# pythoncrazy/jimm

Measured on NVIDIA H100. Metric: images/sec, higher is better.
Workload: dtype f16

## Files before the change

jimm_b200/csrc/common.cuh:

```cuda
#pragma once

#include <cuda.h>
#include <cuda_bf16.h>
#include <cuda_fp16.h>
#include <cuda_runtime.h>
#include <stdint.h>

namespace jimm {

void set_last_error(const char* fmt, ...);

#define JIMM_CUDA_CHECK(expr)                                                                   \
  do {                                                                                          \
    cudaError_t _e = (expr);                                                                    \
    if (_e != cudaSuccess) {                                                                    \
      ::jimm::set_last_error("%s:%d: %s -> %s", __FILE__, __LINE__, #expr, cudaGetErrorString(_e)); \
      return -2;                                                                                \
    }                                                                                           \
  } while (0)

void note_launch();
#define JIMM_LAUNCH_CHECK()                  \
  do {                                       \
    JIMM_CUDA_CHECK(cudaGetLastError());     \
// ... 156 lines not shown
}
__device__ __forceinline__ void mbar_arrive_cluster(uint32_t cluster_addr) {
  asm volatile("mbarrier.arrive.release.cluster.shared::cluster.b64 _, [%0];" ::"r"(cluster_addr) : "memory");
}
__device__ __forceinline__ uint64_t make_wgmma_desc_sw128(uint32_t smem_addr) {
  uint64_t d = 0;
  d |= static_cast<uint64_t>((smem_addr & 0x3FFFFu) >> 4);
  d |= static_cast<uint64_t>(1) << 16;
  d |= static_cast<uint64_t>(1024 >> 4) << 32;
  d |= static_cast<uint64_t>(1) << 62;
  return d;
}
template <int SW>
__device__ __forceinline__ uint64_t make_wgmma_desc(uint32_t smem_addr, uint32_t lbo) {
  static_assert(SW == 128 || SW == 64 || SW == 32, "swizzle width");
  constexpr uint64_t layout = SW == 128 ? 1 : SW == 64 ? 2 : 3;
  uint64_t d = 0;
  d |= static_cast<uint64_t>((smem_addr & 0x3FFFFu) >> 4);
  d |= static_cast<uint64_t>((lbo >> 4) & 0x3FFFu) << 16;
  d |= static_cast<uint64_t>(8 * SW >> 4) << 32;
  d |= layout << 62;
  return d;
}
__device__ __forceinline__ void wgmma_fence() { asm volatile("wgmma.fence.sync.aligned;" ::: "memory"); }
__device__ __forceinline__ void wgmma_commit() { asm volatile("wgmma.commit_group.sync.aligned;" ::: "memory"); }
template <int N>
__device__ __forceinline__ void wgmma_wait() { asm volatile("wgmma.wait_group.sync.aligned %0;" ::"n"(N) : "memory"); }
template <int R>
__device__ __forceinline__ void wgmma_fence_operands(float (&d)[R]) {
#pragma unroll
  for (int i = 0; i < R; ++i) asm volatile("" : "+f"(d[i])::"memory");
}

template <int KIND>
__device__ __forceinline__ void wgmma_m64n128_ss(float (&d)[64], uint64_t adesc, uint64_t bdesc, uint32_t accumulate) {
  if constexpr (KIND == 0) {
    asm volatile(
        "{\n\t.reg .pred p;\n\t"
        "setp.ne.b32 p, %66, 0;\n\t"
        "wgmma.mma_async.sync.aligned.m64n128k16.f32.f16.f16 {%0, %1, %2, %3, %4, %5, %6, %7, %8, %9, %10, %11, %12, %13, %14, %15, %16, %17, %18, %19, %20, %21, %22, %23, %24, %25, %26, %27, %28, %29, %30, %31, %32, %33, %34, %35, %36, %37, %38, %39, %40, %41, %42, %43, %44, %45, %46, %47, %48, %49, %50, %51, %52, %53, %54, %55, %56, %57, %58, %59, %60, %61, %62, %63}, %64, %65, p, 1, 1, 0, 0;\n\t}"
        : "+f"(d[0]), "+f"(d[1]), "+f"(d[2]), "+f"(d[3]), "+f"(d[4]), "+f"(d[5]), "+f"(d[6]), "+f"(d[7]),
          "+f"(d[8]), "+f"(d[9]), "+f"(d[10]), "+f"(d[11]), "+f"(d[12]), "+f"(d[13]), "+f"(d[14]), "+f"(d[15]),
          "+f"(d[16]), "+f"(d[17]), "+f"(d[18]), "+f"(d[19]), "+f"(d[20]), "+f"(d[21]), "+f"(d[22]), "+f"(d[23]),
          "+f"(d[24]), "+f"(d[25]), "+f"(d[26]), "+f"(d[27]), "+f"(d[28]), "+f"(d[29]), "+f"(d[30]), "+f"(d[31]),
          "+f"(d[32]), "+f"(d[33]), "+f"(d[34]), "+f"(d[35]), "+f"(d[36]), "+f"(d[37]), "+f"(d[38]), "+f"(d[39]),
          "+f"(d[40]), "+f"(d[41]), "+f"(d[42]), "+f"(d[43]), "+f"(d[44]), "+f"(d[45]), "+f"(d[46]), "+f"(d[47]),
          "+f"(d[48]), "+f"(d[49]), "+f"(d[50]), "+f"(d[51]), "+f"(d[52]), "+f"(d[53]), "+f"(d[54]), "+f"(d[55]),
          "+f"(d[56]), "+f"(d[57]), "+f"(d[58]), "+f"(d[59]), "+f"(d[60]), "+f"(d[61]), "+f"(d[62]), "+f"(d[63])
        : "l"(adesc), "l"(bdesc), "r"(accumulate));
  } else if constexpr (KIND == 1) {
    asm volatile(
        "{\n\t.reg .pred p;\n\t"
        "setp.ne.b32 p, %66, 0;\n\t"
        "wgmma.mma_async.sync.aligned.m64n128k16.f32.bf16.bf16 {%0, %1, %2, %3, %4, %5, %6, %7, %8, %9, %10, %11, %12, %13, %14, %15, %16, %17, %18, %19, %20, %21, %22, %23, %24, %25, %26, %27, %28, %29, %30, %31, %32, %33, %34, %35, %36, %37, %38, %39, %40, %41, %42, %43, %44, %45, %46, %47, %48, %49, %50, %51, %52, %53, %54, %55, %56, %57, %58, %59, %60, %61, %62, %63}, %64, %65, p, 1, 1, 0, 0;\n\t}"
        : "+f"(d[0]), "+f"(d[1]), "+f"(d[2]), "+f"(d[3]), "+f"(d[4]), "+f"(d[5]), "+f"(d[6]), "+f"(d[7]),
          "+f"(d[8]), "+f"(d[9]), "+f"(d[10]), "+f"(d[11]), "+f"(d[12]), "+f"(d[13]), "+f"(d[14]), "+f"(d[15]),
          "+f"(d[16]), "+f"(d[17]), "+f"(d[18]), "+f"(d[19]), "+f"(d[20]), "+f"(d[21]), "+f"(d[22]), "+f"(d[23]),
          "+f"(d[24]), "+f"(d[25]), "+f"(d[26]), "+f"(d[27]), "+f"(d[28]), "+f"(d[29]), "+f"(d[30]), "+f"(d[31]),
          "+f"(d[32]), "+f"(d[33]), "+f"(d[34]), "+f"(d[35]), "+f"(d[36]), "+f"(d[37]), "+f"(d[38]), "+f"(d[39]),
          "+f"(d[40]), "+f"(d[41]), "+f"(d[42]), "+f"(d[43]), "+f"(d[44]), "+f"(d[45]), "+f"(d[46]), "+f"(d[47]),
          "+f"(d[48]), "+f"(d[49]), "+f"(d[50]), "+f"(d[51]), "+f"(d[52]), "+f"(d[53]), "+f"(d[54]), "+f"(d[55]),
          "+f"(d[56]), "+f"(d[57]), "+f"(d[58]), "+f"(d[59]), "+f"(d[60]), "+f"(d[61]), "+f"(d[62]), "+f"(d[63])
        : "l"(adesc), "l"(bdesc), "r"(accumulate));
  } else {
    asm volatile(
        "{\n\t.reg .pred p;\n\t"
        "setp.ne.b32 p, %66, 0;\n\t"
        "wgmma.mma_async.sync.aligned.m64n128k8.f32.tf32.tf32 {%0, %1, %2, %3, %4, %5, %6, %7, %8, %9, %10, %11, %12, %13, %14, %15, %16, %17, %18, %19, %20, %21, %22, %23, %24, %25, %26, %27, %28, %29, %30, %31, %32, %33, %34, %35, %36, %37, %38, %39, %40, %41, %42, %43, %44, %45, %46, %47, %48, %49, %50, %51, %52, %53, %54, %55, %56, %57, %58, %59, %60, %61, %62, %63}, %64, %65, p, 1, 1;\n\t}"
        : "+f"(d[0]), "+f"(d[1]), "+f"(d[2]), "+f"(d[3]), "+f"(d[4]), "+f"(d[5]), "+f"(d[6]), "+f"(d[7]),
          "+f"(d[8]), "+f"(d[9]), "+f"(d[10]), "+f"(d[11]), "+f"(d[12]), "+f"(d[13]), "+f"(d[14]), "+f"(d[15]),
          "+f"(d[16]), "+f"(d[17]), "+f"(d[18]), "+f"(d[19]), "+f"(d[20]), "+f"(d[21]), "+f"(d[22]), "+f"(d[23]),
          "+f"(d[24]), "+f"(d[25]), "+f"(d[26]), "+f"(d[27]), "+f"(d[28]), "+f"(d[29]), "+f"(d[30]), "+f"(d[31]),
          "+f"(d[32]), "+f"(d[33]), "+f"(d[34]), "+f"(d[35]), "+f"(d[36]), "+f"(d[37]), "+f"(d[38]), "+f"(d[39]),
          "+f"(d[40]), "+f"(d[41]), "+f"(d[42]), "+f"(d[43]), "+f"(d[44]), "+f"(d[45]), "+f"(d[46]), "+f"(d[47]),
          "+f"(d[48]), "+f"(d[49]), "+f"(d[50]), "+f"(d[51]), "+f"(d[52]), "+f"(d[53]), "+f"(d[54]), "+f"(d[55]),
          "+f"(d[56]), "+f"(d[57]), "+f"(d[58]), "+f"(d[59]), "+f"(d[60]), "+f"(d[61]), "+f"(d[62]), "+f"(d[63])
        : "l"(adesc), "l"(bdesc), "r"(accumulate));
  }
}

template <bool BF16>
__device__ __forceinline__ void wgmma_m64n64k16_ss(float (&d)[32], uint64_t adesc, uint64_t bdesc, uint32_t accumulate) {
  if constexpr (BF16) {
    asm volatile(
        "{\n\t.reg .pred p;\n\t"
        "setp.ne.b32 p, %34, 0;\n\t"
        "wgmma.mma_async.sync.aligned.m64n64k16.f32.bf16.bf16 {%0, %1, %2, %3, %4, %5, %6, %7, %8, %9, %10, %11, %12, %13, %14, %15, %16, %17, %18, %19, %20, %21, %22, %23, %24, %25, %26, %27, %28, %29, %30, %31}, %32, %33, p, 1, 1, 0, 0;\n\t}"
        : "+f"(d[0]), "+f"(d[1]), "+f"(d[2]), "+f"(d[3]), "+f"(d[4]), "+f"(d[5]), "+f"(d[6]), "+f"(d[7]),
          "+f"(d[8]), "+f"(d[9]), "+f"(d[10]), "+f"(d[11]), "+f"(d[12]), "+f"(d[13]), "+f"(d[14]), "+f"(d[15]),
          "+f"(d[16]), "+f"(d[17]), "+f"(d[18]), "+f"(d[19]), "+f"(d[20]), "+f"(d[21]), "+f"(d[22]), "+f"(d[23]),
          "+f"(d[24]), "+f"(d[25]), "+f"(d[26]), "+f"(d[27]), "+f"(d[28]), "+f"(d[29]), "+f"(d[30]), "+f"(d[31])
        : "l"(adesc), "l"(bdesc), "r"(accumulate));
  } else {
    asm volatile(
        "{\n\t.reg .pred p;\n\t"
        "setp.ne.b32 p, %34, 0;\n\t"
        "wgmma.mma_async.sync.aligned.m64n64k16.f32.f16.f16 {%0, %1, %2, %3, %4, %5, %6, %7, %8, %9, %10, %11, %12, %13, %14, %15, %16, %17, %18, %19, %20, %21, %22, %23, %24, %25, %26, %27, %28, %29, %30, %31}, %32, %33, p, 1, 1, 0, 0;\n\t}"
        : "+f"(d[0]), "+f"(d[1]), "+f"(d[2]), "+f"(d[3]), "+f"(d[4]), "+f"(d[5]), "+f"(d[6]), "+f"(d[7]),
          "+f"(d[8]), "+f"(d[9]), "+f"(d[10]), "+f"(d[11]), "+f"(d[12]), "+f"(d[13]), "+f"(d[14]), "+f"(d[15]),
          "+f"(d[16]), "+f"(d[17]), "+f"(d[18]), "+f"(d[19]), "+f"(d[20]), "+f"(d[21]), "+f"(d[22]), "+f"(d[23]),
          "+f"(d[24]), "+f"(d[25]), "+f"(d[26]), "+f"(d[27]), "+f"(d[28]), "+f"(d[29]), "+f"(d[30]), "+f"(d[31])
        : "l"(adesc), "l"(bdesc), "r"(accumulate));
  }
}
template <bool BF16, int N>
__device__ __forceinline__ void wgmma_m64nNk16_rs(float (&d)[N / 2], const uint32_t (&a)[4], uint64_t bdesc) {
  static_assert(N == 16 || N == 32 || N == 64 || N == 80 || N == 96 || N == 128, "no wgmma_m64nNk16_rs wrapper for this N");
  if constexpr (N == 16) {
    if constexpr (BF16) {
      asm volatile(
          "wgmma.mma_async.sync.aligned.m64n16k16.f32.bf16.bf16 {%0, %1, %2, %3, %4, %5, %6, %7}, {%8, %9, %10, %11}, %12, 1, 1, 1, 1;"
// ... 183 lines not shown
```

jimm_b200/csrc/gemm.cu:

```cuda
#include "gemm.cuh"

#include <stdarg.h>
#include <stdio.h>
#include <stdlib.h>
#include <string.h>

#include <type_traits>

#include "common.cuh"

namespace jimm {

static constexpr int BM = 128;
static constexpr int BN = 128;
static constexpr int STAGES = 5;
static constexpr int A_STAGE_BYTES = BM * 128;
static constexpr int B_STAGE_BYTES = BN * 128;
static constexpr int STAGE_BYTES = A_STAGE_BYTES + B_STAGE_BYTES;
static constexpr int EPI_WARPS = 8;
static constexpr int EPI_BOX_ROWS = 16;
static constexpr int EPI_BUF_BYTES = EPI_BOX_ROWS * 128;
static constexpr int EPI_BUFS = 2;
static constexpr int EPI_STAGE_BYTES = EPI_WARPS * EPI_BUFS * EPI_BUF_BYTES;
static constexpr int NUM_THREADS = 384;

enum OutKind : int { OUT_GENERIC = 0, OUT_H16 = 1, OUT_BF16 = 2, OUT_TF32 = 3, OUT_F32_ADD = 4, OUT_F32 = 5 };

struct EpiDev {
  const float* bias;
  const float* rowadd;
  const float* residual;
  void* out;
  int act, ldr, out_type, ldo, rows_in, rows_out, row_off, mode;
  int M, N;
  int reverse;
  int tok_pad, tok_off;
  const float* ln_scale;
  const float* ln_bias;
  void* ln_out;
  int* ln_cnt;
  int ln_out_type, ln_ldo;
  float ln_eps;
};

template <int ACT>
__device__ __forceinline__ float act_ct(float v) {
  if constexpr (ACT == ACT_GELU_TANH) return gelu_tanh(v);
  else if constexpr (ACT == ACT_QUICK_GELU) return quick_gelu(v);
  else return v;
}
__device__ __forceinline__ float apply_act(float v, int act) {
  if (act == ACT_GELU_TANH) return gelu_tanh(v);
  if (act == ACT_QUICK_GELU) return quick_gelu(v);
  return v;
}

__device__ __forceinline__ void remap_row(const EpiDev& e, int row, int& out_row, int& add_row) {
// ... 9 lines not shown

__device__ __forceinline__ void store1(const EpiDev& e, int out_row, int col, float v) {
  size_t off = static_cast<size_t>(out_row) * e.ldo + col;
  if (e.out_type == DT_F32) static_cast<float*>(e.out)[off] = v;
  else if (e.out_type == DT_TF32) static_cast<float*>(e.out)[off] = round_tf32(v);
  else if (e.out_type == DT_F16) static_cast<__half*>(e.out)[off] = __float2half_rn(v);
  else static_cast<__nv_bfloat16*>(e.out)[off] = __float2bfloat16_rn(v);
}

template <typename T>
struct Traits;
template <>
struct Traits<__half> {
  static constexpr int KIND = 0;
};
template <>
struct Traits<__nv_bfloat16> {
  static constexpr int KIND = 1;
};
template <>
struct Traits<float> {
  static constexpr int KIND = 2;
};

static constexpr int ACT_FUSE_LN = 7;
static constexpr int LNQ = 240;
struct LnQueue {
  int head, tail, done, pad;
  int slot[LNQ];
};

template <typename OutT, int NV>
__device__ __forceinline__ void ln_rows_nv(const EpiDev& e, int row0, int lane) {
  constexpr int R0 = 12 / NV;
  constexpr int R = R0 < 1 ? 1 : (R0 > 8 ? 8 : R0);
  constexpr bool DOUBLE = NV <= 9;
  const float inv_d = 1.0f / static_cast<float>(NV * 128);
  const float4* sc = reinterpret_cast<const float4*>(e.ln_scale);
  const float4* bi = reinterpret_cast<const float4*>(e.ln_bias);
  const float* xbase = static_cast<const float*>(e.out);
  const int ldx = e.ldo, ldh = e.ln_ldo;
  const float eps = e.ln_eps;
  OutT* hbase = static_cast<OutT*>(e.ln_out);
  const int rows = min(32, e.M - row0);
  float4 a[R][NV];
  float4 b[DOUBLE ? R : 1][DOUBLE ? NV : 1];
#define JIMM_LN_LOAD(buf, r0_)                                                                                          \
  _Pragma("unroll") for (int i = 0; i < R; ++i) {      \
    const float4* xr = reinterpret_cast<const float4*>(xbase + static_cast<size_t>(row0 + min((r0_) + i, rows - 1)) * ldx); \
    _Pragma("unroll") for (int j = 0; j < NV; ++j) buf[i][j] = __ldcg(xr + lane + 32 * j);                              \
  }
#define JIMM_LN_PROCESS(buf, r0_)                                                                                       \
  _Pragma("unroll") for (int i = 0; i < R; ++i) {                                                                       \
    if ((r0_) + i < rows) {                                                                                             \
      float s = 0.f, s2 = 0.f;                                                                                          \
      _Pragma("unroll") for (int j = 0; j < NV; ++j) {                                                                  \
        const float4 v = buf[i][j];                                                                                     \
        s += v.x + v.y + v.z + v.w;                                                                                     \
        s2 += v.x * v.x + v.y * v.y + v.z * v.z + v.w * v.w;                                                            \
      }                                                                                                                 \
      s = warp_sum(s);                                                                                                  \
      s2 = warp_sum(s2);                                                                                                \
      const float mean = s * inv_d;                                                                                     \
      const float rstd = rsqrtf(fmaxf(s2 * inv_d - mean * mean, 0.0f) + eps);                                           \
      OutT* orow = hbase + static_cast<size_t>(row0 + (r0_) + i) * ldh;                                                 \
      _Pragma("unroll") for (int j = 0; j < NV; ++j) {                                                                  \
        const int idx = lane + 32 * j;                                                                                  \
        const float4 v = buf[i][j], g = __ldg(sc + idx), bb = __ldg(bi + idx);                                          \
        float4 y;                                                                                                       \
// ... 13 lines not shown
      }                                                                                                                 \
    }                                                                                                                   \
  }
  if constexpr (DOUBLE) {
    JIMM_LN_LOAD(a, 0)
#pragma unroll 1
    for (int r0 = 0; r0 < rows; r0 += 2 * R) {
      JIMM_LN_LOAD(b, r0 + R)
      JIMM_LN_PROCESS(a, r0)
      JIMM_LN_LOAD(a, r0 + 2 * R)
      JIMM_LN_PROCESS(b, r0 + R)
    }
  } else {
#pragma unroll 1
    for (int r0 = 0; r0 < rows; r0 += R) {
      JIMM_LN_LOAD(a, r0)
      JIMM_LN_PROCESS(a, r0)
    }
  }
#undef JIMM_LN_LOAD
#undef JIMM_LN_PROCESS
}

template <typename OutT>
__device__ __forceinline__ void ln_rows_dispatch(const EpiDev& e, int row0, int lane) {
  switch (e.N >> 7) {
    case 1: ln_rows_nv<OutT, 1>(e, row0, lane); break;
    case 2: ln_rows_nv<OutT, 2>(e, row0, lane); break;
    case 3: ln_rows_nv<OutT, 3>(e, row0, lane); break;
    case 4: ln_rows_nv<OutT, 4>(e, row0, lane); break;
    case 6: ln_rows_nv<OutT, 6>(e, row0, lane); break;
    case 8: ln_rows_nv<OutT, 8>(e, row0, lane); break;
    case 9: ln_rows_nv<OutT, 9>(e, row0, lane); break;
    case 10: ln_rows_nv<OutT, 10>(e, row0, lane); break;
    case 12: ln_rows_nv<OutT, 12>(e, row0, lane); break;
    default: break;
  }
}

__device__ __forceinline__ void ln_publish(const EpiDev& e, LnQueue* q, int rg, int cols) {
  tma_store_wait_all();
  __threadfence();
  const int old = atomicAdd(e.ln_cnt + rg, cols);
  if (old + cols == 2 * e.N) {
    e.ln_cnt[rg] = 0;
    __threadfence();
    const int t = atomicAdd(&q->tail, 1);
    volatile int* s = &q->slot[t % LNQ];
    while (*s != -1) __nanosleep(64);
    *s = rg;
  }
}

template <typename OutT>
__device__ __forceinline__ void ln_worker(const EpiDev& e, LnQueue* q, int lane) {
  for (;;) {
    int rg = -2;
    if (lane == 0) {
      const int t = atomicAdd(&q->head, 1);
      volatile int* s = &q->slot[t % LNQ];
      for (;;) {
        if (*s >= 0) {
          const int v = atomicExch(&q->slot[t % LNQ], -1);
          if (v >= 0) { rg = v; break; }
        }
        if (*reinterpret_cast<volatile int*>(&q->done) == EPI_WARPS && t >= *reinterpret_cast<volatile int*>(&q->tail)) break;
        __nanosleep(256);
      }
      __threadfence();
    }
    rg = __shfl_sync(0xffffffffu, rg, 0);
    if (rg < 0) return;
    ln_rows_dispatch<OutT>(e, rg * 32, lane);
  }
}

template <int OUT, int ACT>
__device__ __forceinline__ void epilogue_tma(const CUtensorMap* map_c, const EpiDev& epi, const float (&acc)[64], uint8_t* tbuf0, int lane,
                                             int row_base, int n_tile0, uint32_t& box_count) {
  constexpr bool OUT16 = (OUT == OUT_H16 || OUT == OUT_BF16);
  constexpr int ES = OUT16 ? 2 : 4;
  constexpr int COLS_PER_BOX = 128 / ES;
  constexpr int JB = COLS_PER_BOX / 8;
  const int g = lane >> 2, t = lane & 3;
#pragma unroll
  for (int s = 0; s < BN / COLS_PER_BOX; ++s) {
    const int n0 = n_tile0 + s * COLS_PER_BOX;
    if (n0 >= epi.N) break;
    uint8_t* tbuf = tbuf0 + (box_count & (EPI_BUFS - 1)) * EPI_BUF_BYTES;
    ++box_count;
    if (lane == 0) tma_store_wait_read1();
    __syncwarp();
#pragma unroll
    for (int jj = 0; jj < JB; ++jj) {
      const int j = s * JB + jj;
      const int col = n0 + jj * 8 + 2 * t;
      float2 b2 = make_float2(0.f, 0.f);
      if (epi.bias != nullptr && col < epi.N) b2 = __ldg(reinterpret_cast<const float2*>(epi.bias + col));
      const float v0 = act_ct<ACT>(acc[4 * j] + b2.x), v1 = act_ct<ACT>(acc[4 * j + 1] + b2.y);
      const float v2 = act_ct<ACT>(acc[4 * j + 2] + b2.x), v3 = act_ct<ACT>(acc[4 * j + 3] + b2.y);
      const int byte = (jj * 8 + 2 * t) * ES;
      const int off = ((((byte >> 4) ^ g)) << 4) + (byte & 15);
      uint8_t* p0 = tbuf + g * 128 + off;
      uint8_t* p1 = p0 + 8 * 128;
      if constexpr (OUT16) {
        *reinterpret_cast<uint32_t*>(p0) = pack2(v0, v1, OUT == OUT_H16 ? 1 : 2);
        *reinterpret_cast<uint32_t*>(p1) = pack2(v2, v3, OUT == OUT_H16 ? 1 : 2);
      } else if constexpr (OUT == OUT_TF32) {
        *reinterpret_cast<float2*>(p0) = make_float2(round_tf32(v0), round_tf32(v1));
        *reinterpret_cast<float2*>(p1) = make_float2(round_tf32(v2), round_tf32(v3));
      } else {
        *reinterpret_cast<float2*>(p0) = make_float2(v0, v1);
        *reinterpret_cast<float2*>(p1) = make_float2(v2, v3);
      }
    }
    fence_proxy_async_smem();
    __syncwarp();
    if (lane == 0) {
      const uint32_t tbuf_u32 = smem_u32(tbuf);
      if constexpr (OUT == OUT_F32_ADD) {
        if (epi.tok_pad > 0) {
          const int b = row_base / epi.tok_pad;
          tma_reduce_add_3d(map_c, tbuf_u32, n0, row_base - b * epi.tok_pad + epi.tok_off, b);
        } else {
          tma_reduce_add_2d(map_c, tbuf_u32, n0, row_base);
        }
      } else {
        tma_store_2d(map_c, tbuf_u32, n0, row_base);
      }
      tma_store_commit();
    }
  }
}

__device__ __forceinline__ void epilogue_generic(const EpiDev& epi, const float (&acc)[64], int lane, int row_base, int n_tile0) {
  const int g = lane >> 2, t = lane & 3;
#pragma unroll
  for (int h = 0; h < 2; ++h) {
    const int row = row_base + g + 8 * h;
    if (row >= epi.M) continue;
    int out_row, add_row;
    remap_row(epi, row, out_row, add_row);
#pragma unroll
    for (int j = 0; j < BN / 8; ++j) {
#pragma unroll
      for (int q = 0; q < 2; ++q) {
        const int col = n_tile0 + 8 * j + 2 * t + q;
        if (col < epi.N) {
          float v = acc[4 * j + 2 * h + q];
          if (epi.bias) v += __ldg(epi.bias + col);
          v = apply_act(v, epi.act);
          if (epi.rowadd) v += __ldg(epi.rowadd + static_cast<size_t>(add_row) * epi.N + col);
          if (epi.residual) v += epi.residual[static_cast<size_t>(out_row) * epi.ldr + col];
          store1(epi, out_row, col, v);
        }
      }
    }
  }
}

template <typename T, int OUT, int ACT>
__global__ void __launch_bounds__(NUM_THREADS, 1)
gemm_wgmma_kernel(const __grid_constant__ CUtensorMap map_a, const __grid_constant__ CUtensorMap map_b,
                  const __grid_constant__ CUtensorMap map_c, const EpiDev epi, int K) {
  constexpr int BK = 128 / sizeof(T);
  constexpr int UK = 32 / sizeof(T);
  constexpr bool FUSE_LN = OUT == OUT_F32_ADD && ACT == ACT_FUSE_LN;
  constexpr int EPI_ACT = ACT == ACT_FUSE_LN ? static_cast<int>(ACT_NONE) : ACT;

  extern __shared__ uint8_t smem_raw[];
  uint8_t* smem = reinterpret_cast<uint8_t*>((reinterpret_cast<uintptr_t>(smem_raw) + 1023) & ~static_cast<uintptr_t>(1023));
  uint8_t* smem_a = smem;
  uint8_t* smem_b = smem + STAGES * A_STAGE_BYTES;
  uint8_t* epi_stage = smem + STAGES * STAGE_BYTES;
  LnQueue* lnq = reinterpret_cast<LnQueue*>(epi_stage + EPI_STAGE_BYTES);
  uint64_t* full_bar = reinterpret_cast<uint64_t*>(lnq + 1);
  uint64_t* empty_bar = full_bar + STAGES;

  const int warp_idx = threadIdx.x >> 5;
  const int lane = threadIdx.x & 31;
  const int M = epi.M, N = epi.N;
  const int m_tiles = (M + BM - 1) / BM, n_tiles = (N + BN - 1) / BN;
  const int num_tiles = m_tiles * n_tiles;
  const int num_kb = (K + BK - 1) / BK;

  pdl_launch_dependents();
  if (warp_idx == 0 && lane == 0) {
    tma_prefetch_desc(&map_a);
    tma_prefetch_desc(&map_b);
    if constexpr (OUT != OUT_GENERIC) tma_prefetch_desc(&map_c);
    for (int s = 0; s < STAGES; ++s) {
      mbar_init(&full_bar[s], 1);
      mbar_init(&empty_bar[s], EPI_WARPS);
    }
    fence_barrier_init();
  }
  if constexpr (FUSE_LN) {
    if (warp_idx == 1) {
      for (int i = lane; i < LNQ; i += 32) lnq->slot[i] = -1;
      if (lane == 0) lnq->head = lnq->tail = lnq->done = 0;
    }
  }
  __syncthreads();
  pdl_wait();

  if (warp_idx < 4) {
    if (warp_idx == 0) {
      if (lane == 0) {
        int stage = 0;
        uint32_t phase = 0;
        for (int tile = blockIdx.x; tile < num_tiles; tile += gridDim.x) {
          const int tv = epi.reverse ? num_tiles - 1 - tile : tile;
          const int m_blk = tv / n_tiles, n_blk = tv - m_blk * n_tiles;
          for (int kb = 0; kb < num_kb; ++kb) {
            mbar_wait(&empty_bar[stage], phase ^ 1);
            mbar_arrive_expect_tx(&full_bar[stage], STAGE_BYTES);
            tma_load_2d(smem_a + stage * A_STAGE_BYTES, &map_a, &full_bar[stage], kb * BK, m_blk * BM);
            tma_load_2d(smem_b + stage * B_STAGE_BYTES, &map_b, &full_bar[stage], kb * BK, n_blk * BN);
            if (++stage == STAGES) { stage = 0; phase ^= 1; }
          }
        }
      }
    } else if constexpr (FUSE_LN) {
      ln_worker<T>(epi, lnq, lane);
    }
  } else {
    const int wg = (warp_idx - 4) >> 2;
    const int wq = warp_idx & 3;
    uint8_t* tbuf0 = epi_stage + (warp_idx - 4) * EPI_BUFS * EPI_BUF_BYTES;
    int stage = 0;
    uint32_t phase = 0, box_count = 0;
    int ln_rg = -1, ln_cols = 0;
    float acc[64];
    for (int tile = blockIdx.x; tile < num_tiles; tile += gridDim.x) {
      const int tv = epi.reverse ? num_tiles - 1 - tile : tile;
      const int m_blk = tv / n_tiles, n_blk = tv - m_blk * n_tiles;
      int prev = -1;
      for (int kb = 0; kb < num_kb; ++kb) {
        mbar_wait(&full_bar[stage], phase);
        const uint64_t adesc = make_wgmma_desc_sw128(smem_u32(smem_a + stage * A_STAGE_BYTES + wg * 64 * 128));
        const uint64_t bdesc = make_wgmma_desc_sw128(smem_u32(smem_b + stage * B_STAGE_BYTES));
        wgmma_fence_operands(acc);
        wgmma_fence();
#pragma unroll
        for (int k = 0; k < BK / UK; ++k)
          wgmma_m64n128_ss<Traits<T>::KIND>(acc, adesc + static_cast<uint64_t>(2 * k), bdesc + static_cast<uint64_t>(2 * k), (kb | k) != 0 ? 1u : 0u);
        wgmma_commit();
        wgmma_fence_operands(acc);
        if (prev >= 0) {
          wgmma_wait<1>();
          if (lane == 0) mbar_arrive(&empty_bar[prev]);
        }
        prev = stage;
        if (++stage == STAGES) { stage = 0; phase ^= 1; }
      }
      wgmma_wait<0>();
      wgmma_fence_operands(acc);
      if (lane == 0) mbar_arrive(&empty_bar[prev]);

      const int row_base = m_blk * BM + wg * 64 + wq * 16;
      const int n_tile0 = n_blk * BN;
      if constexpr (OUT == OUT_GENERIC) {
        epilogue_generic(epi, acc, lane, row_base, n_tile0);
      } else {
        if (row_base < M) epilogue_tma<OUT, EPI_ACT>(&map_c, epi, acc, tbuf0, lane, row_base, n_tile0, box_count);
        if constexpr (FUSE_LN) {
          if (lane == 0 && ln_rg >= 0) ln_publish(epi, lnq, ln_rg, ln_cols);
          ln_rg = (row_base & ~31) < M ? row_base >> 5 : -1;
          ln_cols = min(BN, N - n_tile0);
        }
      }
    }
    if constexpr (FUSE_LN) {
      if (lane == 0) {
        if (ln_rg >= 0) ln_publish(epi, lnq, ln_rg, ln_cols);
        __threadfence_block();
        atomicAdd(&lnq->done, 1);
      }
    }
// ... 142 lines not shown
                    (epi.bias == nullptr || ((reinterpret_cast<uintptr_t>(epi.bias) & 15) == 0 && N % 4 == 0)) &&
                    !(epi.residual && epi.act != ACT_NONE);
    if (ok && epi.tok_pad > 0) {
      if (int rc = make_map_3d_f32(&plan->map_c, epi.out, M / epi.tok_pad, epi.tok_S, N, epi.ldo)) return rc;
    } else if (ok) {
      if (int rc = make_map(&plan->map_c, epi.out_type, epi.out, M, N, epi.ldo, EPI_BOX_ROWS)) return rc;
    } else {
      plan->epi.mode = 0;
    }
  }
  if (epi.tok_pad > 0 && plan->epi.mode != 2) {
    set_last_error("gemm: the token scatter needs the TMA epilogue (mode 2, no activation, 16-byte aligned output / bias, N %% 4 == 0)");
    return -1;
  }
  return 0;
}

static EpiDev to_dev(const GemmEpilogue& e, int M, int N) {
  EpiDev d;
  d.bias = e.bias; d.rowadd = e.rowadd; d.residual = e.residual; d.out = e.out;
  d.act = e.act; d.ldr = e.ldr; d.out_type = e.out_type; d.ldo = e.ldo;
  d.rows_in = e.rows_in; d.rows_out = e.rows_out; d.row_off = e.row_off; d.mode = e.mode;
  d.M = M; d.N = N;
  d.tok_pad = e.tok_pad; d.tok_off = e.tok_off;
  d.reverse = e.reverse;
  d.ln_scale = e.ln_scale; d.ln_bias = e.ln_bias; d.ln_out = e.ln_out; d.ln_cnt = e.ln_cnt;
  d.ln_out_type = e.ln_out_type; d.ln_ldo = e.ln_ldo; d.ln_eps = e.ln_eps;
  return d;
}

template <typename T, int OUT, int ACT>
static int launch_one(const GemmPlan* p, int M, cudaStream_t stream) {
  static DeviceOnce attr_set;
  if (attr_set.first()) JIMM_CUDA_CHECK(cudaFuncSetAttribute(gemm_wgmma_kernel<T, OUT, ACT>, cudaFuncAttributeMaxDynamicSharedMemorySize, SMEM_BYTES));
  const int tiles = ((M + BM - 1) / BM) * ((p->N + BN - 1) / BN);
  const int grid = tiles < device_sm_count() ? tiles : device_sm_count();
  JIMM_CUDA_CHECK(launch_k(gemm_wgmma_kernel<T, OUT, ACT>, dim3(grid), dim3(NUM_THREADS), SMEM_BYTES, stream, 1, true, p->map_a, p->map_b,
                           p->map_c, to_dev(p->epi, M, p->N), p->K));
  note_launch();
  return 0;
}

template <typename T, int OUT>
static int launch_act(const GemmPlan* p, int M, cudaStream_t stream) {
  switch (p->epi.act) {
    case ACT_GELU_TANH: return launch_one<T, OUT, ACT_GELU_TANH>(p, M, stream);
    case ACT_QUICK_GELU: return launch_one<T, OUT, ACT_QUICK_GELU>(p, M, stream);
    default: return launch_one<T, OUT, ACT_NONE>(p, M, stream);
  }
}

template <typename T>
static int launch_tc(const GemmPlan* p, int M, cudaStream_t stream) {
  const GemmEpilogue& e = p->epi;
  if (e.mode != 2) return launch_one<T, OUT_GENERIC, ACT_NONE>(p, M, stream);
  if (e.residual) return gemm_fuses_ln(p, M) ? launch_one<T, OUT_F32_ADD, ACT_FUSE_LN>(p, M, stream) : launch_one<T, OUT_F32_ADD, ACT_NONE>(p, M, stream);
  switch (e.out_type) {
    case DT_F16: return launch_act<T, OUT_H16>(p, M, stream);
    case DT_BF16: return launch_act<T, OUT_BF16>(p, M, stream);
    case DT_TF32: return launch_act<T, OUT_TF32>(p, M, stream);
    default: return launch_act<T, OUT_F32>(p, M, stream);
  }
}

int gemm_fuses_ln(const GemmPlan* p, int ) {
  const int nv = p->N >> 7;
  const bool width_ok = p->N % 128 == 0 && (nv <= 4 || nv == 6 || (nv >= 8 && nv <= 10) || nv == 12);
  const int want = p->dtype == DT_F16 ? DT_F16 : p->dtype == DT_BF16 ? DT_BF16 : DT_TF32;
  return p->epi.ln_cnt != nullptr && p->epi.ln_out_type == want && width_ok && p->epi.mode == 2 && p->epi.residual != nullptr && p->epi.tok_pad == 0;
}

int gemm_plan_run(const GemmPlan* p0, int M_override, cudaStream_t stream, int reverse) {
  const int M = (M_override > 0 && M_override <= p0->M) ? M_override : p0->M;
  if (p0->epi.tok_pad > 0 && M % p0->epi.tok_pad != 0) {
    set_last_error("gemm: token scatter runs whole samples (M=%d, tok_pad=%d)", M, p0->epi.tok_pad);
    return -1;
  }
  GemmPlan local;
  const GemmPlan* p = p0;
  if (reverse != p0->epi.reverse) { local = *p0; local.epi.reverse = reverse; p = &local; }
  switch (p->dtype) {
    case DT_F16: return launch_tc<__half>(p, M, stream);
    case DT_BF16: return launch_tc<__nv_bfloat16>(p, M, stream);
    case DT_F32:
    case DT_TF32: return launch_tc<float>(p, M, stream);
  }
  set_last_error("gemm: bad dtype %d", p->dtype);
  return -1;
}

int gemm_simt_run(int dtype, const void* A, int lda, const void* B, int ldb, int M, int N, int K, const GemmEpilogue& epi,
                  cudaStream_t stream) {
  if (int rc = check_epi(epi, N)) return rc;
  dim3 block(16, 16), grid((N + 15) / 16, (M + 15) / 16);
  EpiDev d = to_dev(epi, M, N);
  if (dtype == DT_F16) gemm_simt_kernel<__half><<<grid, block, 0, stream>>>(static_cast<const __half*>(A), lda, static_cast<const __half*>(B), ldb, K, d);
  else if (dtype == DT_BF16) gemm_simt_kernel<__nv_bfloat16><<<grid, block, 0, stream>>>(static_cast<const __nv_bfloat16*>(A), lda, static_cast<const __nv_bfloat16*>(B), ldb, K, d);
  else gemm_simt_kernel<float><<<grid, block, 0, stream>>>(static_cast<const float*>(A), lda, static_cast<const float*>(B), ldb, K, d);
  JIMM_LAUNCH_CHECK();
  return 0;
// ... 4 lines not shown
```

jimm_b200/csrc/gemm.cuh:

```cuda
#pragma once
#include <cuda.h>
#include <cuda_runtime.h>
#include <stdint.h>

namespace jimm {

enum DType : int { DT_F32 = 0, DT_F16 = 1, DT_BF16 = 2, DT_TF32 = 3 };
enum Act : int { ACT_NONE = 0, ACT_GELU_TANH = 1, ACT_QUICK_GELU = 2 };

inline size_t dtype_size(int dt) { return (dt == DT_F32 || dt == DT_TF32) ? 4 : 2; }

struct GemmEpilogue {
  const float* bias = nullptr;
  int act = ACT_NONE;
  const float* rowadd = nullptr;
  const float* residual = nullptr;
  int ldr = 0;
  void* out = nullptr;
  int out_type = DT_F32;
  int ldo = 0;
  int tok_pad = 0, tok_off = 0, tok_S = 0;
  int reverse = 0;
  int rows_in = 0, rows_out = 0, row_off = 0;
  int mode = 2;
  const float* ln_scale = nullptr;
  const float* ln_bias = nullptr;
  void* ln_out = nullptr;
  int ln_out_type = DT_F16, ln_ldo = 0;
  float ln_eps = 1e-6f;
  int* ln_cnt = nullptr;
};

struct GemmPlan {
  CUtensorMap map_a, map_b, map_c;
  int M = 0, N = 0, K = 0;
  int dtype = DT_F16;
  GemmEpilogue epi;
};

int gemm_plan_init(GemmPlan* plan, int dtype, const void* A, int lda, const void* B, int ldb, int M, int N, int K,
                   const GemmEpilogue& epi);
int gemm_plan_run(const GemmPlan* plan, int M_override, cudaStream_t stream, int reverse = 0);

// ... 9 lines not shown
```

jimm_b200/csrc/model.cu:

```cuda
#include <stdarg.h>
#include <stdio.h>
#include <stdlib.h>
#include <string.h>

#include <atomic>
#include <cmath>
#include <map>
#include <tuple>
#include <memory>
#include <string>
#include <vector>

#include "../../include/jimm_b200.h"
#include "comm.cuh"
#include "common.cuh"
#include "gemm.cuh"
#include "kernels.cuh"

namespace jimm {

static thread_local char g_err[1024] = "";
void set_last_error(const char* fmt, ...) {
  va_list ap;
  va_start(ap, fmt);
// ... 1086 lines not shown
  if (m->copy_stream) return 0;
  JIMM_CUDA_CHECK(cudaStreamCreateWithFlags(&m->copy_stream, cudaStreamNonBlocking));
  for (int i = 0; i < jimm_model::kHostSlices; ++i) {
    JIMM_CUDA_CHECK(cudaEventCreateWithFlags(&m->ev_copied[i], cudaEventDisableTiming));
    JIMM_CUDA_CHECK(cudaEventCreateWithFlags(&m->ev_consumed[i], cudaEventDisableTiming));
  }
  JIMM_CUDA_CHECK(cudaEventCreateWithFlags(&m->ev_start, cudaEventDisableTiming));
  return 0;
}

static void host_slices(const jimm_model* m, int nb, int* sizes, size_t bytes_per_image = 0) {
  for (int i = 0; i < jimm_model::kHostSlices; ++i) sizes[i] = 0;
  sizes[0] = nb;
  if (const char* env = getenv("JIMM_HOST_SLICES")) {
    int k = 0, acc = 0;
    for (const char* q = env; *q && k < jimm_model::kHostSlices - 1;) {
      const int v = atoi(q);
      if (v <= 0 || acc + v >= nb) break;
      sizes[k++] = v;
      acc += v;
      while (*q && *q != ',') ++q;
      if (*q == ',') ++q;
    }
    sizes[k] = nb - acc;
    return;
  }
  if (nb < 128) return;
  if (bytes_per_image && static_cast<size_t>(nb) * bytes_per_image < (static_cast<size_t>(64) << 20)) return;
  static int head_div = -1;
  if (head_div < 0) { const char* env = getenv("JIMM_HOST_HEAD_DIV"); head_div = (env && atoi(env) > 0) ? atoi(env) : 4; }
  const int S = m->vis.S, D = m->vis.D, Mm = m->vis.enc.c.M;
  const int sms = device_sm_count();
  auto cost = [&](int n) {
    const long mt = (static_cast<long>(n) * S + 127) / 128;
    auto rounds = [&](int N) { return (mt * ((N + 127) / 128) + sms - 1) / sms; };
    return static_cast<double>(D) * rounds(3 * D) + static_cast<double>(D) * rounds(D) + static_cast<double>(D) * rounds(Mm) +
           static_cast<double>(Mm) * rounds(D);
  };
  int best = nb / head_div;
  double best_cost = 1e30;
  for (int c0 = nb / head_div; c0 <= nb / 3; ++c0) {
    const double cst = cost(c0) + cost(nb - c0) + 1e-3 * c0 * D;
    if (cst < best_cost) { best_cost = cst; best = c0; }
  }
  sizes[0] = best;
  sizes[1] = nb - best;
}

static int vit_forward_host_impl(jimm_model_t* m, const void* img_host, int in_dtype, int B, float* out_host, cudaStream_t s,
                                 jimm_preproc_t* pre, int Hin, int Win) {
  JIMM_TRY(ensure_copy_stream(m));
  const size_t img_elems = static_cast<size_t>(m->vis.img) * m->vis.img * m->vis.C;
  const size_t src_bytes = pre ? static_cast<size_t>(Hin) * Win * 3 : img_elems * dtype_size(in_dtype);
  const int tower_dtype = pre ? (m->cdt == DT_TF32 ? JIMM_F32 : m->cdt) : in_dtype;
  const int od = vision_out_dim(m);
  const int kind = pre ? 1 : 0;
  if (pre) {
    const size_t need = static_cast<size_t>(m->max_batch) * src_bytes;
    if (need > m->ws.in_u8_bytes) {
      JIMM_CUDA_CHECK(cudaDeviceSynchronize());
      if (m->ws.in_u8) cudaFree(m->ws.in_u8);
      m->ws.in_u8 = nullptr; m->ws.in_u8_bytes = 0;
      JIMM_CUDA_CHECK(cudaMalloc(&m->ws.in_u8, need));
      m->ws.in_u8_bytes = need;
      m->host_chain = false;
    }
  }
  for (int b0 = 0; b0 < B; b0 += m->max_batch) {
// ... 159 lines not shown
  }
  if (gemm_ms) *gemm_ms = ms;
  if (gemm_flops) *gemm_flops = m->prof_flops;
  if (gemm_launches) *gemm_launches = m->prof_launches;
  m->prof_used = 0;
  return 0;
}

int jimm_k_gemm_ex(int impl, int dtype, const void* A, int lda, const void* B, int ldb, int M, int N, int K, const float* bias, int act,
                   const float* rowadd, const float* residual, int ldr, void* out, int out_type, int ldo, int rows_in, int rows_out,
                   int row_off, int epi_mode, int plan_M, int reverse, int tok_pad, int tok_off, int tok_S, const float* ln_scale,
                   const float* ln_bias, float ln_eps, void* ln_out, int ln_out_type, int ln_ldo, int* ln_counters, void* stream) {
  if (plan_M <= 0) plan_M = M;
  if (M <= 0 || M > plan_M) { set_last_error("jimm_k_gemm_ex: need 0 < M <= plan_M (M=%d plan_M=%d)", M, plan_M); return JIMM_EINVAL; }
  GemmEpilogue e;
  e.bias = bias; e.act = act; e.rowadd = rowadd; e.residual = residual; e.ldr = ldr; e.out = out; e.out_type = out_type; e.ldo = ldo;
  e.rows_in = rows_in; e.rows_out = rows_out; e.row_off = row_off; e.mode = epi_mode;
  e.tok_pad = tok_pad; e.tok_off = tok_off; e.tok_S = tok_S;
  if (ln_counters) {
    e.ln_scale = ln_scale; e.ln_bias = ln_bias; e.ln_out = ln_out; e.ln_out_type = ln_out_type == JIMM_F32 ? DT_TF32 : ln_out_type; e.ln_ldo = ln_ldo;
    e.ln_eps = ln_eps; e.ln_cnt = ln_counters;
  }
  cudaStream_t s = static_cast<cudaStream_t>(stream);
  if (impl == 1) {
    if (plan_M != M || reverse || tok_pad || ln_counters) {
      set_last_error("jimm_k_gemm_ex: the SIMT GEMM has no plan rows, reverse walk, token scatter or fused LayerNorm");
      return JIMM_EINVAL;
    }
    return gemm_simt_run(dtype, A, lda, B, ldb, M, N, K, e, s);
  }
  GemmPlan p;
  JIMM_TRY(gemm_plan_init(&p, dtype, A, lda, B, ldb, plan_M, N, K, e));
  if (ln_counters && !gemm_fuses_ln(&p, M)) {
    set_last_error("gemm: this shape does not take the fused LayerNorm path (needs N = 128 x {1,2,3,4,6,8,9,10,12}, aligned operands, "
                   "LayerNorm output in the operand type)");
    return JIMM_EINVAL;
  }
  return gemm_plan_run(&p, M, s, reverse);
}
int jimm_k_gemm(int impl, int dtype, const void* A, int lda, const void* B, int ldb, int M, int N, int K, const float* bias, int act,
                const float* rowadd, const float* residual, int ldr, void* out, int out_type, int ldo, int rows_in, int rows_out,
                int row_off, int epi_mode, void* stream) {
  return jimm_k_gemm_ex(impl, dtype, A, lda, B, ldb, M, N, K, bias, act, rowadd, residual, ldr, out, out_type, ldo, rows_in, rows_out, row_off,
                        epi_mode, M, 0, 0, 0, 0, nullptr, nullptr, 0.f, nullptr, 0, 0, nullptr, stream);
}
int jimm_k_gemm_residual_ln(int dtype, const void* A, int lda, const void* B, int ldb, int M, int N, int K, const float* bias, float* x, int ldx,
                            const float* ln_scale, const float* ln_bias, float eps, void* ln_out, int ln_out_type, int ln_ldo, int* counters,
                            void* stream) {
  if (!counters) { set_last_error("jimm_k_gemm_residual_ln: null counters"); return JIMM_EINVAL; }
  return jimm_k_gemm_ex(0, dtype, A, lda, B, ldb, M, N, K, bias, 0, nullptr, x, ldx, x, JIMM_F32, ldx, 0, 0, 0, 2, M, 0, 0, 0, 0, ln_scale,
                        ln_bias, eps, ln_out, ln_out_type, ln_ldo, counters, stream);
}
int jimm_k_layernorm_ex(const float* x, int ldx, int group, int row_off, const int32_t* row_index, const float* scale, const float* bias,
                        float eps, void* out, int out_type, int ldy, int rows, int D, int reverse, void* stream) {
  return layernorm_run(x, ldx, group, row_off, row_index, scale, bias, eps, out, out_type, ldy, rows, D, static_cast<cudaStream_t>(stream), reverse);
}
int jimm_k_layernorm(const float* x, int ldx, int group, int row_off, const int32_t* row_index, const float* scale, const float* bias,
                     float eps, void* out, int out_type, int ldy, int rows, int D, void* stream) {
  return jimm_k_layernorm_ex(x, ldx, group, row_off, row_index, scale, bias, eps, out, out_type, ldy, rows, D, 0, stream);
}
int jimm_k_attention_hd(const void* qkv, int io_type, void* out, int out_type, int B, int S, int H, int head_dim, int causal, int reverse,
                        void* stream) {
  return attention_run(qkv, io_type, out, out_type, B, S, H, head_dim, causal, static_cast<cudaStream_t>(stream), reverse);
}
int jimm_k_attention_ex(const void* qkv, int io_type, void* out, int out_type, int B, int S, int H, int causal, int reverse, void* stream) {
  return jimm_k_attention_hd(qkv, io_type, out, out_type, B, S, H, 64, causal, reverse, stream);
}
// ... 33 lines not shown
```

Measured before the change: 8857.

## Widen GEMM tiles to 128x256 with m64n256 wgmma and setmaxnreg register split

Switches the persistent wgmma GEMM from 128x128 to 128x256 tiles, using m64n256 wgmma instructions with 128-float accumulators per consumer thread. Pipeline stages drop from 5 to 4 to fit shared memory, and setmaxnreg moves registers from the producer warpgroup to the consumer warpgroups. The aim is higher operand reuse per loaded byte and fewer wgmma issues. In exchange, the grid has fewer tiles, which can cause wave quantization on narrow GEMMs. The fused-LayerNorm widths 10 and 12 are dropped, and launch now fails if the kernel is not compiled to exactly 168 registers.

```diff
diff --git a/jimm_b200/csrc/common.cuh b/jimm_b200/csrc/common.cuh
--- a/jimm_b200/csrc/common.cuh
+++ b/jimm_b200/csrc/common.cuh
@@ -212,51 +212,45 @@
   for (int i = 0; i < R; ++i) asm volatile("" : "+f"(d[i])::"memory");
 }
 
+#define JIMM_WGMMA_D128                                                                                                                    \
+  "{%0, %1, %2, %3, %4, %5, %6, %7, %8, %9, %10, %11, %12, %13, %14, %15, %16, %17, %18, %19, %20, %21, %22, %23, %24, %25, %26, %27, "     \
+  "%28, %29, %30, %31, %32, %33, %34, %35, %36, %37, %38, %39, %40, %41, %42, %43, %44, %45, %46, %47, %48, %49, %50, %51, %52, %53, %54, " \
+  "%55, %56, %57, %58, %59, %60, %61, %62, %63, %64, %65, %66, %67, %68, %69, %70, %71, %72, %73, %74, %75, %76, %77, %78, %79, %80, %81, " \
+  "%82, %83, %84, %85, %86, %87, %88, %89, %90, %91, %92, %93, %94, %95, %96, %97, %98, %99, %100, %101, %102, %103, %104, %105, %106, "   \
+  "%107, %108, %109, %110, %111, %112, %113, %114, %115, %116, %117, %118, %119, %120, %121, %122, %123, %124, %125, %126, %127}"
+#define JIMM_WGMMA_D8(i) "+f"(d[i]), "+f"(d[i + 1]), "+f"(d[i + 2]), "+f"(d[i + 3]), "+f"(d[i + 4]), "+f"(d[i + 5]), "+f"(d[i + 6]), "+f"(d[i + 7])
+#define JIMM_WGMMA_D128_OPERANDS                                                                                                 \
+  JIMM_WGMMA_D8(0), JIMM_WGMMA_D8(8), JIMM_WGMMA_D8(16), JIMM_WGMMA_D8(24), JIMM_WGMMA_D8(32), JIMM_WGMMA_D8(40), JIMM_WGMMA_D8(48), \
+      JIMM_WGMMA_D8(56), JIMM_WGMMA_D8(64), JIMM_WGMMA_D8(72), JIMM_WGMMA_D8(80), JIMM_WGMMA_D8(88), JIMM_WGMMA_D8(96),             \
+      JIMM_WGMMA_D8(104), JIMM_WGMMA_D8(112), JIMM_WGMMA_D8(120)
 template <int KIND>
-__device__ __forceinline__ void wgmma_m64n128_ss(float (&d)[64], uint64_t adesc, uint64_t bdesc, uint32_t accumulate) {
+__device__ __forceinline__ void wgmma_m64n256_ss(float (&d)[128], uint64_t adesc, uint64_t bdesc, uint32_t accumulate) {
   if constexpr (KIND == 0) {
-    asm volatile(
-        "{\n\t.reg .pred p;\n\t"
-        "setp.ne.b32 p, %66, 0;\n\t"
-        "wgmma.mma_async.sync.aligned.m64n128k16.f32.f16.f16 {%0, %1, %2, %3, %4, %5, %6, %7, %8, %9, %10, %11, %12, %13, %14, %15, %16, %17, %18, %19, %20, %21, %22, %23, %24, %25, %26, %27, %28, %29, %30, %31, %32, %33, %34, %35, %36, %37, %38, %39, %40, %41, %42, %43, %44, %45, %46, %47, %48, %49, %50, %51, %52, %53, %54, %55, %56, %57, %58, %59, %60, %61, %62, %63}, %64, %65, p, 1, 1, 0, 0;\n\t}"
-        : "+f"(d[0]), "+f"(d[1]), "+f"(d[2]), "+f"(d[3]), "+f"(d[4]), "+f"(d[5]), "+f"(d[6]), "+f"(d[7]),
-          "+f"(d[8]), "+f"(d[9]), "+f"(d[10]), "+f"(d[11]), "+f"(d[12]), "+f"(d[13]), "+f"(d[14]), "+f"(d[15]),
-          "+f"(d[16]), "+f"(d[17]), "+f"(d[18]), "+f"(d[19]), "+f"(d[20]), "+f"(d[21]), "+f"(d[22]), "+f"(d[23]),
-          "+f"(d[24]), "+f"(d[25]), "+f"(d[26]), "+f"(d[27]), "+f"(d[28]), "+f"(d[29]), "+f"(d[30]), "+f"(d[31]),
-          "+f"(d[32]), "+f"(d[33]), "+f"(d[34]), "+f"(d[35]), "+f"(d[36]), "+f"(d[37]), "+f"(d[38]), "+f"(d[39]),
-          "+f"(d[40]), "+f"(d[41]), "+f"(d[42]), "+f"(d[43]), "+f"(d[44]), "+f"(d[45]), "+f"(d[46]), "+f"(d[47]),
-          "+f"(d[48]), "+f"(d[49]), "+f"(d[50]), "+f"(d[51]), "+f"(d[52]), "+f"(d[53]), "+f"(d[54]), "+f"(d[55]),
-          "+f"(d[56]), "+f"(d[57]), "+f"(d[58]), "+f"(d[59]), "+f"(d[60]), "+f"(d[61]), "+f"(d[62]), "+f"(d[63])
-        : "l"(adesc), "l"(bdesc), "r"(accumulate));
+    asm volatile("{\n\t.reg .pred p;\n\tsetp.ne.b32 p, %130, 0;\n\t"
+                 "wgmma.mma_async.sync.aligned.m64n256k16.f32.f16.f16 " JIMM_WGMMA_D128 ", %128, %129, p, 1, 1, 0, 0;\n\t}"
+                 : JIMM_WGMMA_D128_OPERANDS
+                 : "l"(adesc), "l"(bdesc), "r"(accumulate));
   } else if constexpr (KIND == 1) {
-    asm volatile(
-        "{\n\t.reg .pred p;\n\t"
-        "setp.ne.b32 p, %66, 0;\n\t"
-        "wgmma.mma_async.sync.aligned.m64n128k16.f32.bf16.bf16 {%0, %1, %2, %3, %4, %5, %6, %7, %8, %9, %10, %11, %12, %13, %14, %15, %16, %17, %18, %19, %20, %21, %22, %23, %24, %25, %26, %27, %28, %29, %30, %31, %32, %33, %34, %35, %36, %37, %38, %39, %40, %41, %42, %43, %44, %45, %46, %47, %48, %49, %50, %51, %52, %53, %54, %55, %56, %57, %58, %59, %60, %61, %62, %63}, %64, %65, p, 1, 1, 0, 0;\n\t}"
-        : "+f"(d[0]), "+f"(d[1]), "+f"(d[2]), "+f"(d[3]), "+f"(d[4]), "+f"(d[5]), "+f"(d[6]), "+f"(d[7]),
-          "+f"(d[8]), "+f"(d[9]), "+f"(d[10]), "+f"(d[11]), "+f"(d[12]), "+f"(d[13]), "+f"(d[14]), "+f"(d[15]),
-          "+f"(d[16]), "+f"(d[17]), "+f"(d[18]), "+f"(d[19]), "+f"(d[20]), "+f"(d[21]), "+f"(d[22]), "+f"(d[23]),
-          "+f"(d[24]), "+f"(d[25]), "+f"(d[26]), "+f"(d[27]), "+f"(d[28]), "+f"(d[29]), "+f"(d[30]), "+f"(d[31]),
-          "+f"(d[32]), "+f"(d[33]), "+f"(d[34]), "+f"(d[35]), "+f"(d[36]), "+f"(d[37]), "+f"(d[38]), "+f"(d[39]),
-          "+f"(d[40]), "+f"(d[41]), "+f"(d[42]), "+f"(d[43]), "+f"(d[44]), "+f"(d[45]), "+f"(d[46]), "+f"(d[47]),
-          "+f"(d[48]), "+f"(d[49]), "+f"(d[50]), "+f"(d[51]), "+f"(d[52]), "+f"(d[53]), "+f"(d[54]), "+f"(d[55]),
-          "+f"(d[56]), "+f"(d[57]), "+f"(d[58]), "+f"(d[59]), "+f"(d[60]), "+f"(d[61]), "+f"(d[62]), "+f"(d[63])
-        : "l"(adesc), "l"(bdesc), "r"(accumulate));
+    asm volatile("{\n\t.reg .pred p;\n\tsetp.ne.b32 p, %130, 0;\n\t"
+                 "wgmma.mma_async.sync.aligned.m64n256k16.f32.bf16.bf16 " JIMM_WGMMA_D128 ", %128, %129, p, 1, 1, 0, 0;\n\t}"
+                 : JIMM_WGMMA_D128_OPERANDS
+                 : "l"(adesc), "l"(bdesc), "r"(accumulate));
   } else {
-    asm volatile(
-        "{\n\t.reg .pred p;\n\t"
-        "setp.ne.b32 p, %66, 0;\n\t"
-        "wgmma.mma_async.sync.aligned.m64n128k8.f32.tf32.tf32 {%0, %1, %2, %3, %4, %5, %6, %7, %8, %9, %10, %11, %12, %13, %14, %15, %16, %17, %18, %19, %20, %21, %22, %23, %24, %25, %26, %27, %28, %29, %30, %31, %32, %33, %34, %35, %36, %37, %38, %39, %40, %41, %42, %43, %44, %45, %46, %47, %48, %49, %50, %51, %52, %53, %54, %55, %56, %57, %58, %59, %60, %61, %62, %63}, %64, %65, p, 1, 1;\n\t}"
-        : "+f"(d[0]), "+f"(d[1]), "+f"(d[2]), "+f"(d[3]), "+f"(d[4]), "+f"(d[5]), "+f"(d[6]), "+f"(d[7]),
-          "+f"(d[8]), "+f"(d[9]), "+f"(d[10]), "+f"(d[11]), "+f"(d[12]), "+f"(d[13]), "+f"(d[14]), "+f"(d[15]),
-          "+f"(d[16]), "+f"(d[17]), "+f"(d[18]), "+f"(d[19]), "+f"(d[20]), "+f"(d[21]), "+f"(d[22]), "+f"(d[23]),
-          "+f"(d[24]), "+f"(d[25]), "+f"(d[26]), "+f"(d[27]), "+f"(d[28]), "+f"(d[29]), "+f"(d[30]), "+f"(d[31]),
-          "+f"(d[32]), "+f"(d[33]), "+f"(d[34]), "+f"(d[35]), "+f"(d[36]), "+f"(d[37]), "+f"(d[38]), "+f"(d[39]),
-          "+f"(d[40]), "+f"(d[41]), "+f"(d[42]), "+f"(d[43]), "+f"(d[44]), "+f"(d[45]), "+f"(d[46]), "+f"(d[47]),
-          "+f"(d[48]), "+f"(d[49]), "+f"(d[50]), "+f"(d[51]), "+f"(d[52]), "+f"(d[53]), "+f"(d[54]), "+f"(d[55]),
-          "+f"(d[56]), "+f"(d[57]), "+f"(d[58]), "+f"(d[59]), "+f"(d[60]), "+f"(d[61]), "+f"(d[62]), "+f"(d[63])
-        : "l"(adesc), "l"(bdesc), "r"(accumulate));
-  }
+    asm volatile("{\n\t.reg .pred p;\n\tsetp.ne.b32 p, %130, 0;\n\t"
+                 "wgmma.mma_async.sync.aligned.m64n256k8.f32.tf32.tf32 " JIMM_WGMMA_D128 ", %128, %129, p, 1, 1;\n\t}"
+                 : JIMM_WGMMA_D128_OPERANDS
+                 : "l"(adesc), "l"(bdesc), "r"(accumulate));
+  }
+}
+#undef JIMM_WGMMA_D128
+#undef JIMM_WGMMA_D8
+#undef JIMM_WGMMA_D128_OPERANDS
+
+template <int FROM, int TO>
+__device__ __forceinline__ void setmaxnreg() {
+  static_assert(TO % 8 == 0 && TO >= 24 && TO <= 256, "setmaxnreg takes a multiple of 8 in [24, 256]");
+  if constexpr (TO < FROM) asm volatile("setmaxnreg.dec.sync.aligned.u32 %0;" ::"n"(TO));
+  else if constexpr (TO > FROM) asm volatile("setmaxnreg.inc.sync.aligned.u32 %0;" ::"n"(TO));
 }
 
 template <bool BF16>
diff --git a/jimm_b200/csrc/gemm.cu b/jimm_b200/csrc/gemm.cu
--- a/jimm_b200/csrc/gemm.cu
+++ b/jimm_b200/csrc/gemm.cu
@@ -11,9 +11,10 @@
 
 namespace jimm {
 
-static constexpr int BM = 128;
-static constexpr int BN = 128;
-static constexpr int STAGES = 5;
+static constexpr int BM = GEMM_TILE_M;
+static constexpr int BN = GEMM_TILE_N;
+static_assert(BM == 128 && BN == 256, "the warp roles and the wgmma shape below are written for 128 x 256 tiles");
+static constexpr int STAGES = 4;
 static constexpr int A_STAGE_BYTES = BM * 128;
 static constexpr int B_STAGE_BYTES = BN * 128;
 static constexpr int STAGE_BYTES = A_STAGE_BYTES + B_STAGE_BYTES;
@@ -23,6 +24,7 @@
 static constexpr int EPI_BUFS = 2;
 static constexpr int EPI_STAGE_BYTES = EPI_WARPS * EPI_BUFS * EPI_BUF_BYTES;
 static constexpr int NUM_THREADS = 384;
+static constexpr int KERNEL_REGS = 168;
 
 enum OutKind : int { OUT_GENERIC = 0, OUT_H16 = 1, OUT_BF16 = 2, OUT_TF32 = 3, OUT_F32_ADD = 4, OUT_F32 = 5 };
 
@@ -98,9 +100,9 @@
 
 template <typename OutT, int NV>
 __device__ __forceinline__ void ln_rows_nv(const EpiDev& e, int row0, int lane) {
-  constexpr int R0 = 12 / NV;
-  constexpr int R = R0 < 1 ? 1 : (R0 > 8 ? 8 : R0);
-  constexpr bool DOUBLE = NV <= 9;
+  constexpr int R0 = 8 / NV;
+  constexpr int R = R0 < 1 ? 1 : R0;
+  constexpr bool DOUBLE = NV <= 8;
   const float inv_d = 1.0f / static_cast<float>(NV * 128);
   const float4* sc = reinterpret_cast<const float4*>(e.ln_scale);
   const float4* bi = reinterpret_cast<const float4*>(e.ln_bias);
@@ -180,8 +182,6 @@
     case 6: ln_rows_nv<OutT, 6>(e, row0, lane); break;
     case 8: ln_rows_nv<OutT, 8>(e, row0, lane); break;
     case 9: ln_rows_nv<OutT, 9>(e, row0, lane); break;
-    case 10: ln_rows_nv<OutT, 10>(e, row0, lane); break;
-    case 12: ln_rows_nv<OutT, 12>(e, row0, lane); break;
     default: break;
   }
 }
@@ -224,7 +224,7 @@
 }
 
 template <int OUT, int ACT>
-__device__ __forceinline__ void epilogue_tma(const CUtensorMap* map_c, const EpiDev& epi, const float (&acc)[64], uint8_t* tbuf0, int lane,
+__device__ __forceinline__ void epilogue_tma(const CUtensorMap* map_c, const EpiDev& epi, const float (&acc)[128], uint8_t* tbuf0, int lane,
                                              int row_base, int n_tile0, uint32_t& box_count) {
   constexpr bool OUT16 = (OUT == OUT_H16 || OUT == OUT_BF16);
   constexpr int ES = OUT16 ? 2 : 4;
@@ -281,7 +281,7 @@
   }
 }
 
-__device__ __forceinline__ void epilogue_generic(const EpiDev& epi, const float (&acc)[64], int lane, int row_base, int n_tile0) {
+__device__ __forceinline__ void epilogue_generic(const EpiDev& epi, const float (&acc)[128], int lane, int row_base, int n_tile0) {
   const int g = lane >> 2, t = lane & 3;
 #pragma unroll
   for (int h = 0; h < 2; ++h) {
@@ -315,6 +315,9 @@
   constexpr int UK = 32 / sizeof(T);
   constexpr bool FUSE_LN = OUT == OUT_F32_ADD && ACT == ACT_FUSE_LN;
   constexpr int EPI_ACT = ACT == ACT_FUSE_LN ? static_cast<int>(ACT_NONE) : ACT;
+  constexpr int PRODUCER_REGS = FUSE_LN ? 152 : 40;
+  constexpr int CONSUMER_REGS = FUSE_LN ? 176 : 232;
+  static_assert(128 * PRODUCER_REGS + 256 * CONSUMER_REGS <= NUM_THREADS * KERNEL_REGS, "register split exceeds the CTA's allocation");
 
   extern __shared__ uint8_t smem_raw[];
   uint8_t* smem = reinterpret_cast<uint8_t*>((reinterpret_cast<uintptr_t>(smem_raw) + 1023) & ~static_cast<uintptr_t>(1023));
@@ -353,6 +356,7 @@
   pdl_wait();
 
   if (warp_idx < 4) {
+    setmaxnreg<KERNEL_REGS, PRODUCER_REGS>();
     if (warp_idx == 0) {
       if (lane == 0) {
         int stage = 0;
@@ -373,13 +377,14 @@
       ln_worker<T>(epi, lnq, lane);
     }
   } else {
+    setmaxnreg<KERNEL_REGS, CONSUMER_REGS>();
     const int wg = (warp_idx - 4) >> 2;
     const int wq = warp_idx & 3;
     uint8_t* tbuf0 = epi_stage + (warp_idx - 4) * EPI_BUFS * EPI_BUF_BYTES;
     int stage = 0;
     uint32_t phase = 0, box_count = 0;
     int ln_rg = -1, ln_cols = 0;
-    float acc[64];
+    float acc[128];
     for (int tile = blockIdx.x; tile < num_tiles; tile += gridDim.x) {
       const int tv = epi.reverse ? num_tiles - 1 - tile : tile;
       const int m_blk = tv / n_tiles, n_blk = tv - m_blk * n_tiles;
@@ -392,7 +397,7 @@
         wgmma_fence();
 #pragma unroll
         for (int k = 0; k < BK / UK; ++k)
-          wgmma_m64n128_ss<Traits<T>::KIND>(acc, adesc + static_cast<uint64_t>(2 * k), bdesc + static_cast<uint64_t>(2 * k), (kb | k) != 0 ? 1u : 0u);
+          wgmma_m64n256_ss<Traits<T>::KIND>(acc, adesc + static_cast<uint64_t>(2 * k), bdesc + static_cast<uint64_t>(2 * k), (kb | k) != 0 ? 1u : 0u);
         wgmma_commit();
         wgmma_fence_operands(acc);
         if (prev >= 0) {
@@ -601,7 +606,15 @@
 template <typename T, int OUT, int ACT>
 static int launch_one(const GemmPlan* p, int M, cudaStream_t stream) {
   static DeviceOnce attr_set;
-  if (attr_set.first()) JIMM_CUDA_CHECK(cudaFuncSetAttribute(gemm_wgmma_kernel<T, OUT, ACT>, cudaFuncAttributeMaxDynamicSharedMemorySize, SMEM_BYTES));
+  if (attr_set.first()) {
+    JIMM_CUDA_CHECK(cudaFuncSetAttribute(gemm_wgmma_kernel<T, OUT, ACT>, cudaFuncAttributeMaxDynamicSharedMemorySize, SMEM_BYTES));
+    cudaFuncAttributes fa;
+    JIMM_CUDA_CHECK(cudaFuncGetAttributes(&fa, gemm_wgmma_kernel<T, OUT, ACT>));
+    if (fa.numRegs != KERNEL_REGS) {
+      set_last_error("gemm: kernel compiled with %d registers per thread, the warpgroup register split assumes %d", fa.numRegs, KERNEL_REGS);
+      return -2;
+    }
+  }
   const int tiles = ((M + BM - 1) / BM) * ((p->N + BN - 1) / BN);
   const int grid = tiles < device_sm_count() ? tiles : device_sm_count();
   JIMM_CUDA_CHECK(launch_k(gemm_wgmma_kernel<T, OUT, ACT>, dim3(grid), dim3(NUM_THREADS), SMEM_BYTES, stream, 1, true, p->map_a, p->map_b,
@@ -634,7 +647,7 @@
 
 int gemm_fuses_ln(const GemmPlan* p, int ) {
   const int nv = p->N >> 7;
-  const bool width_ok = p->N % 128 == 0 && (nv <= 4 || nv == 6 || (nv >= 8 && nv <= 10) || nv == 12);
+  const bool width_ok = p->N % 128 == 0 && (nv <= 4 || nv == 6 || nv == 8 || nv == 9);
   const int want = p->dtype == DT_F16 ? DT_F16 : p->dtype == DT_BF16 ? DT_BF16 : DT_TF32;
   return p->epi.ln_cnt != nullptr && p->epi.ln_out_type == want && width_ok && p->epi.mode == 2 && p->epi.residual != nullptr && p->epi.tok_pad == 0;
 }
diff --git a/jimm_b200/csrc/gemm.cuh b/jimm_b200/csrc/gemm.cuh
--- a/jimm_b200/csrc/gemm.cuh
+++ b/jimm_b200/csrc/gemm.cuh
@@ -9,6 +9,9 @@
 enum Act : int { ACT_NONE = 0, ACT_GELU_TANH = 1, ACT_QUICK_GELU = 2 };
 
 inline size_t dtype_size(int dt) { return (dt == DT_F32 || dt == DT_TF32) ? 4 : 2; }
+
+constexpr int GEMM_TILE_M = 128;
+constexpr int GEMM_TILE_N = 256;
 
 struct GemmEpilogue {
   const float* bias = nullptr;
diff --git a/jimm_b200/csrc/model.cu b/jimm_b200/csrc/model.cu
--- a/jimm_b200/csrc/model.cu
+++ b/jimm_b200/csrc/model.cu
@@ -1142,8 +1142,8 @@
   const int S = m->vis.S, D = m->vis.D, Mm = m->vis.enc.c.M;
   const int sms = device_sm_count();
   auto cost = [&](int n) {
-    const long mt = (static_cast<long>(n) * S + 127) / 128;
-    auto rounds = [&](int N) { return (mt * ((N + 127) / 128) + sms - 1) / sms; };
+    const long mt = (static_cast<long>(n) * S + GEMM_TILE_M - 1) / GEMM_TILE_M;
+    auto rounds = [&](int N) { return (mt * ((N + GEMM_TILE_N - 1) / GEMM_TILE_N) + sms - 1) / sms; };
     return static_cast<double>(D) * rounds(3 * D) + static_cast<double>(D) * rounds(D) + static_cast<double>(D) * rounds(Mm) +
            static_cast<double>(Mm) * rounds(D);
   };
@@ -1369,7 +1369,7 @@
   GemmPlan p;
   JIMM_TRY(gemm_plan_init(&p, dtype, A, lda, B, ldb, plan_M, N, K, e));
   if (ln_counters && !gemm_fuses_ln(&p, M)) {
-    set_last_error("gemm: this shape does not take the fused LayerNorm path (needs N = 128 x {1,2,3,4,6,8,9,10,12}, aligned operands, "
+    set_last_error("gemm: this shape does not take the fused LayerNorm path (needs N = 128 x {1,2,3,4,6,8,9}, aligned operands, "
                    "LayerNorm output in the operand type)");
     return JIMM_EINVAL;
   }
```

After: 9617, median of 6. 8.6% higher.
